# eniac/otti

Hardware: AMD Instinct MI355X
Metric: R1CS constraints/sec proved (Spartan NIZK) at 2^20 (higher is better)
Workload: dtype u256 (GF(l) / GF(2^255-19), 8 x u32 limbs)

## Files before the change

### include/otti_spartan.h

```cpp
#ifndef OTTI_SPARTAN_H
#define OTTI_SPARTAN_H
#include <stdint.h>
#include <stddef.h>

#ifdef __cplusplus
extern "C" {
#endif

enum {
    OTTI_OK = 0,
    OTTI_ERR_NON_POW2_CONS = -1,
    OTTI_ERR_NON_POW2_VARS = -2,
    OTTI_ERR_INVALID_NUM_INPUTS = -3,
    OTTI_ERR_INVALID_NUM_VARS = -4,
    OTTI_ERR_INVALID_SCALAR = -5,
    OTTI_ERR_INVALID_INDEX = -6,
    OTTI_ERR_VERIFY_INTERNAL = -10,
    OTTI_ERR_VERIFY_DECOMPRESS = -11,
    OTTI_ERR_MALFORMED_PROOF = -12,
    OTTI_ERR_NO_DEVICE = -20,
    OTTI_ERR_BAD_ARG = -21,
    OTTI_ERR_IO = -22,
    OTTI_ERR_INTERNAL = -23
};
// ... 123 lines not shown
                              uint8_t *io_Az, uint8_t *io_Bz, uint8_t *io_Cz, uint64_t *io_bits, uint64_t *io_unsat,
                              uint32_t *h_rows, size_t n_rows_cap, uint64_t *n_touched, int32_t *took_full_pass, float *kernel_ms);
int32_t otti_k_eval_table_sparse(otti_instance *inst, const uint8_t *h_eq_rx, const uint8_t *h_rABC , uint8_t *h_out, float *kernel_ms);
typedef struct { uint64_t rows, entries[3], n_heavy, n_seg; int32_t use_small, quad; } otti_device_info;
int32_t otti_instance_device_info(otti_instance *inst, int32_t by_col, otti_device_info *out);
int32_t otti_k_eq_evals(const uint8_t *h_r, size_t ell, uint8_t *h_out, float *kernel_ms);
int32_t otti_k_fold_top(const uint8_t *h_Z, size_t len, const uint8_t *h_r, uint8_t *h_out, float *kernel_ms);
int32_t otti_k_fold_bot(const uint8_t *h_Z, size_t len, const uint8_t *h_r, uint8_t *h_out, float *kernel_ms);
int32_t otti_k_sc_cubic_round(const uint8_t *h_A, const uint8_t *h_B, const uint8_t *h_C, const uint8_t *h_D, size_t len, uint8_t *h_e3, float *kernel_ms);
int32_t otti_k_sc_cubic_fold_round(const uint8_t *h_A, const uint8_t *h_B, const uint8_t *h_C, const uint8_t *h_D, size_t len,
                                   const uint8_t *h_r, uint8_t *h_out4, uint8_t *h_e3, float *kernel_ms);
int32_t otti_k_sc_quad_round(const uint8_t *h_A, const uint8_t *h_B, size_t len, uint8_t *h_e2, float *kernel_ms);
int32_t otti_k_sc_quad_fold_round(const uint8_t *h_A, const uint8_t *h_B, size_t len, const uint8_t *h_r, uint8_t *h_out2, uint8_t *h_e2, float *kernel_ms);
int32_t otti_k_armed_selftest(const uint8_t *A, const uint8_t *B, size_t len, const uint8_t *r, uint32_t hold_us, uint8_t *out2, uint8_t *e2);
int32_t otti_k_msm_rows(otti_gens *gens, const uint8_t *h_Z, size_t L, size_t R, const uint8_t *h_blinds, uint8_t *h_out32, float *kernel_ms);
int32_t otti_k_msm_scatter_rows(otti_gens *gens, size_t L, const uint64_t *h_idx, const uint8_t *h_s, size_t count,
                                uint8_t *h_out32, float *kernel_ms);
int32_t otti_k_witness_diff(const uint8_t *h_old, size_t n, const void *h_src, int32_t format, size_t stride_bytes, uint8_t *h_new,
                            uint64_t *h_idx, uint8_t *h_delta, uint64_t *n_changed, uint32_t *chunk, float *kernel_ms);
int32_t otti_k_row_sum(const uint8_t *h_compressed32, size_t n, const uint8_t *h_scalars_mont32, uint8_t *h_out32);

int32_t otti_k_eq_pyramid(const uint8_t *h_r, size_t n, uint8_t *h_out);
int32_t otti_k_sc_cubic3_round(const uint8_t *h_B, const uint8_t *h_C, const uint8_t *h_D, size_t len, const uint8_t *h_tau, uint8_t *h_e3, float *kernel_ms);
int32_t otti_k_sc_cubic3_fold_round(const uint8_t *h_B, const uint8_t *h_C, const uint8_t *h_D, size_t len, const uint8_t *h_r, const uint8_t *h_tau,
                                    uint8_t *h_out3, uint8_t *h_e3, float *kernel_ms);
int32_t otti_k_poly_bound(const uint8_t *h_Z, size_t L, size_t R, const uint8_t *h_Lv, uint8_t *h_out, float *kernel_ms);
int32_t otti_k_bullet_round(otti_gens *gens, size_t n_cur, int32_t fold, const uint8_t *h_u, const uint8_t *h_uinv, const uint8_t *h_a, const uint8_t *h_b,
                            const uint8_t *h_s, const uint8_t *h_blinds2, uint8_t *h_a_out, uint8_t *h_b_out, uint8_t *h_s_out, uint8_t *h_LR64, float *kernel_ms);
int32_t otti_k_bullet_last_fold(size_t R, const uint8_t *h_u, const uint8_t *h_uinv, uint8_t *h_a2, uint8_t *h_b2, uint8_t *h_s);
int32_t otti_k_pc_round(const uint8_t *h_A, const uint8_t *h_B, const uint8_t *h_C, const uint8_t *h_has_C, size_t ninst, size_t len, const uint8_t *h_tau,
// ... 48 lines not shown
```

### otti_amd/api.py

```python
import contextlib
import ctypes
import os
import sys
import numpy as np

L_ORDER = 2 ** 252 + 27742317777372353535851937790883648493
_R = (1 << 256) % L_ORDER
_RINV = pow(_R, -1, L_ORDER)

ENTRY_DTYPE = np.dtype([("row", "<u8"), ("col", "<u8"), ("val", "u1", (32,))])

_HERE = os.path.dirname(os.path.abspath(__file__))
lib_path = os.path.join(_HERE, "libottispartan.so")


class SpartanError(Exception):
    def __init__(self, code, msg=""):
        super().__init__(f"{type(self).__name__}({code}): {msg}")
        self.code = code


class R1CSError(SpartanError):
    """upstream R1CSError: InvalidNumberOfInputs(-3) InvalidNumberOfVars(-4) InvalidScalar(-5) InvalidIndex(-6)"""

# ... 122 lines not shown
_sig("otti_k_addr_timestamps", _i32, _vp, _sz, _sz, _vp, _vp, _fp)
_sig("otti_k_fr_to_canonical", _i32, _vp, _vp, _sz)
_sig("otti_k_multiply_vec", _i32, _vp, _vp, _vp, _vp, _vp, _fp)
_sig("otti_k_eval_table_sparse", _i32, _vp, _vp, _vp, _vp, _fp)
_sig("otti_k_products_patch", _i32, _vp, _vp, _vp, _sz, _sz, _sz, _vp, _vp, _vp, _vp, ctypes.POINTER(_u64), _vp, _sz, ctypes.POINTER(_u64), ctypes.POINTER(_i32), _fp)
_sig("otti_instance_device_info", _i32, _vp, _i32, ctypes.POINTER(_DeviceInfo))
_sig("otti_k_eq_evals", _i32, _vp, _sz, _vp, _fp)
_sig("otti_k_fold_top", _i32, _vp, _sz, _vp, _vp, _fp)
_sig("otti_k_fold_bot", _i32, _vp, _sz, _vp, _vp, _fp)
_sig("otti_k_sc_cubic_round", _i32, _vp, _vp, _vp, _vp, _sz, _vp, _fp)
_sig("otti_k_sc_cubic_fold_round", _i32, _vp, _vp, _vp, _vp, _sz, _vp, _vp, _vp, _fp)
_sig("otti_k_sc_quad_round", _i32, _vp, _vp, _sz, _vp, _fp)
_sig("otti_k_sc_quad_fold_round", _i32, _vp, _vp, _sz, _vp, _vp, _vp, _fp)
_sig("otti_k_armed_selftest", _i32, _vp, _vp, _sz, _vp, ctypes.c_uint32, _vp, _vp)
_sig("otti_k_msm_rows", _i32, _vp, _vp, _sz, _sz, _vp, _vp, _fp)
_sig("otti_k_row_sum", _i32, _vp, _sz, _vp, _vp)
_sig("otti_k_msm_scatter_rows", _i32, _vp, _sz, _vp, _vp, _sz, _vp, _fp)
_sig("otti_k_witness_diff", _i32, _vp, _sz, _vp, _i32, _sz, _vp, _vp, _vp, ctypes.POINTER(_u64), ctypes.POINTER(ctypes.c_uint32), _fp)
_sig("otti_k_eq_pyramid", _i32, _vp, _sz, _vp)
_sig("otti_k_sc_cubic3_round", _i32, _vp, _vp, _vp, _sz, _vp, _vp, _fp)
_sig("otti_k_sc_cubic3_fold_round", _i32, _vp, _vp, _vp, _sz, _vp, _vp, _vp, _vp, _fp)
_sig("otti_k_poly_bound", _i32, _vp, _sz, _sz, _vp, _vp, _fp)
_sig("otti_k_bullet_round", _i32, _vp, _sz, _i32, _vp, _vp, _vp, _vp, _vp, _vp, _vp, _vp, _vp, _vp, _fp)
_sig("otti_k_bullet_last_fold", _i32, _sz, _vp, _vp, _vp, _vp, _vp)
_u32 = ctypes.c_uint32
_sig("otti_k_pc_round", _i32, _vp, _vp, _vp, _vp, _sz, _sz, _vp, _vp, _u32, _u32, _vp, _vp, _fp)
_sig("otti_k_pc_export", _i32, _vp, _vp, _vp, _vp, _sz, _sz, _vp, _vp)
_sig("otti_k_pc_tail", _i32, _vp, _vp, _vp, _vp, _sz, _sz, _u32, _sz, _vp, _vp, _vp, _i32, _vp, _vp)
_sig("otti_k_prod_layer", _i32, _vp, _vp, _sz, _sz, _vp, _vp, _fp)
_sig("otti_k_hash_mem", _i32, _vp, _vp, _sz, _vp, _vp, _u32, _u32, _vp, _vp, _fp)
# ... 884 lines not shown
            raise ValueError("src is shorter than n elements at this stride")
        new, idx, delta = np.zeros((n, 32), dtype=np.uint8), np.zeros(n, dtype=np.uint64), np.zeros((n, 32), dtype=np.uint8)
        k, chunk = _u64(), ctypes.c_uint32()
        _check(lib.otti_k_witness_diff(_ptr(old), n, _ptr(raw), fmt, stride_bytes, _ptr(new), _ptr(idx), _ptr(delta), ctypes.byref(k), ctypes.byref(chunk), None))
        return new, idx[:k.value].copy(), delta[:k.value].copy(), chunk.value

    @staticmethod
    def msm_rows(gens, Z, L, R, blinds):
        Z, blinds = _scalars(Z, "Z"), _scalars(blinds, "blinds")
        assert Z.shape[0] == L * R and blinds.shape[0] == L
        out = np.zeros((L, 32), dtype=np.uint8); ms = ctypes.c_float(0)
        _check(lib.otti_k_msm_rows(gens._h, _ptr(Z), L, R, _ptr(blinds), _ptr(out), ctypes.byref(ms)))
        return out, ms.value

    @staticmethod
    def eq_pyramid(r):
        r = _scalars(r, "r"); n = r.shape[0]
        out = np.zeros(((2 << n) - 1, 32), dtype=np.uint8)
        _check(lib.otti_k_eq_pyramid(_ptr(r), n, _ptr(out)))
        return out

    @staticmethod
    def sc_cubic3_round(B, C, D, tau):
        B, C, D, tau = (_scalars(x, "t") for x in (B, C, D, tau)); e = np.zeros((3, 32), dtype=np.uint8); ms = ctypes.c_float(0)
        assert (1 << (tau.shape[0] + 1)) == B.shape[0]
        _check(lib.otti_k_sc_cubic3_round(_ptr(B), _ptr(C), _ptr(D), B.shape[0], _ptr(tau), _ptr(e), ctypes.byref(ms)))
        return e, ms.value

    @staticmethod
    def sc_cubic3_fold_round(B, C, D, r, tau):
# ... 232 lines not shown
```

### otti_amd/csrc/capi_kernels.cpp

```cpp
#include "capi_common.h"

namespace {
struct Staged {
    DevBuf<Fr> d;
    Staged(DevCtx &c, const uint8_t *h, size_t n) : d(std::max<size_t>(1, n)) { if (n) OTTI_HIP(hipMemcpyAsync(d.p, h, n * sizeof(Fr), hipMemcpyHostToDevice, c.stream)); }
};
void download(DevCtx &c, uint8_t *h, const Fr *d, size_t n) { if (n) OTTI_HIP(hipMemcpyAsync(h, d, n * sizeof(Fr), hipMemcpyDeviceToHost, c.stream)); }
struct KTimer {
    DevCtx &c; float *out;
    KTimer(DevCtx &c_, float *o) : c(c_), out(o) { if (out) OTTI_HIP(hipEventRecord(c.ev0, c.stream)); }
    void stop() { if (out) { OTTI_HIP(hipEventRecord(c.ev1, c.stream)); OTTI_HIP(hipEventSynchronize(c.ev1)); OTTI_HIP(hipEventElapsedTime(out, c.ev0, c.ev1)); } }
};
struct EqPyramids {
    DevBuf<Fr> buf; size_t n_lo = 0, n_hi = 0;
    EqPyramids(DevCtx &c, const Fr *tau, size_t m) : buf(8192 + 16384) {
        n_lo = std::min<size_t>(m, 12); n_hi = m - n_lo;
        dev_eq_pyramid2(c, tau + n_hi, n_lo, buf.p, tau, n_hi, n_hi ? buf.p + 8192 : nullptr);
    }
    EqSrc top() const {
        EqSrc e; const size_t m = n_lo + n_hi;
        if (m <= n_lo) { e.hi = nullptr; e.lo = buf.p + (((size_t)1 << m) - 1); e.lo_bits = 0; }
        else { e.hi = buf.p + 8192 + (((size_t)1 << n_hi) - 1); e.lo = buf.p + (((size_t)1 << n_lo) - 1); e.lo_bits = (int)n_lo; }
        return e;
    }
// ... 235 lines not shown
        pt_encode(out32, sum); return OTTI_OK;
    });
}
int32_t otti_k_msm_rows(otti_gens *gens, const uint8_t *Z, size_t L, size_t R, const uint8_t *blinds, uint8_t *out32, float *ms) {
    return guarded([&] {
        DevCtx &c = DevCtx::get(); Gens &g = *gens->g;
        if (R != g.R) throw Error(OTTI_ERR_BAD_ARG, "row length differs from the generator count");
        ensure_gens_device(g);
        Staged z(c, Z, L * R), bl(c, blinds, L);
        uint32_t hb = g.pc_n.h;
        const bool sparse = dev_small_fraction(c, z.d.p, L * R) > kSparseWitness;
        KTimer t(c, ms); dev_msm_rows(c, *g.dev, {.dense = z.d.p, .n_dense = R, .rows = L, .extra_s = bl.d.p, .extra_base = &hb, .n_extra = 1, .sparse = sparse}); t.stop();
        c.sync(); memcpy(out32, c.h_points, 32 * L); return OTTI_OK;
    });
}

int32_t otti_k_msm_scatter_rows(otti_gens *gens, size_t L, const uint64_t *idx, const uint8_t *s, size_t count, uint8_t *out32, float *ms) {
    return guarded([&] {
        if (!gens || !out32 || !L || L > 4096 || (count && (!idx || !s))) throw Error(OTTI_ERR_BAD_ARG, "null argument, or L outside 1 .. 4096");
        Gens &g = *gens->g;
        for (size_t i = 0; i < count; i++)
            if (idx[i] >= L * g.R || (i && idx[i] <= idx[i - 1])) throw Error(OTTI_ERR_INVALID_INDEX, "the indices are not strictly ascending below L * R");
        DevCtx &c = DevCtx::get();
        ensure_gens_device(g);
        Staged sc(c, s, count);
        DevBuf<uint64_t> d_idx(std::max<size_t>(1, count)); DevBuf<Pt> rows(L); DevBuf<uint8_t> enc(32 * L);
        const std::vector<Pt> id(L, pt_identity());
        if (count) OTTI_HIP(hipMemcpyAsync(d_idx.p, idx, count * sizeof(uint64_t), hipMemcpyHostToDevice, c.stream));
        OTTI_HIP(hipMemcpyAsync(rows.p, id.data(), L * sizeof(Pt), hipMemcpyHostToDevice, c.stream));
        KTimer t(c, ms); dev_msm_scatter(c, *g.dev, d_idx.p, sc.d.p, count, g.R, rows.p, L); t.stop();
// ... 358 lines not shown
```

### otti_amd/csrc/device.h

```cpp
#pragma once
#include <hip/hip_runtime.h>
#include <vector>
#include <functional>
#include <cstddef>
#include <chrono>
#include "spartan.h"
#include "mail.h"
#include "msm_plan.h"
#include "sc_plan.h"

namespace otti {

#define OTTI_HIP(expr) ::otti::hip_check((expr), #expr, __FILE__, __LINE__)
void hip_check(hipError_t e, const char *what, const char *file, int line);
struct OutOfDeviceMemory : Error { using Error::Error; };
struct TailTimeout : Error { using Error::Error; };

template <class T> struct DevBuf {
    T *p = nullptr; size_t n = 0;
    DevBuf() {}
    explicit DevBuf(size_t count) { alloc(count); }
    DevBuf(const DevBuf &) = delete; DevBuf &operator=(const DevBuf &) = delete;
    DevBuf(DevBuf &&o) noexcept : p(o.p), n(o.n) { o.p = nullptr; o.n = 0; }
    DevBuf &operator=(DevBuf &&o) noexcept { if (this != &o) { release(); p = o.p; n = o.n; o.p = nullptr; o.n = 0; } return *this; }
// ... 233 lines not shown
void dev_fold_bot(DevCtx &c, const Fr *Z, Fr *out, size_t len, const Fr &r);
void dev_fetch(DevCtx &c, const Fr *src, int slot, size_t n);
struct MsmJob {
    const Fr *dense = nullptr; size_t n_dense = 0, rows = 0;
    const Fr *extra_s = nullptr; const uint32_t *extra_base = nullptr ; size_t n_extra = 0;
    int mode = MSM_COMPRESSED;
    const Pt *addend = nullptr;
    bool sparse = false;
    Pt *keep_dst = nullptr; bool force_bulk = false;
};
constexpr double kSparseWitness = 0.25;
MsmTicket dev_msm_rows(DevCtx &c, const DeviceGens &g, const MsmJob &job);
double dev_small_fraction(DevCtx &c, const Fr *z, size_t n);
void dev_msm_scatter(DevCtx &c, const DeviceGens &g, const uint64_t *d_idx, const Fr *d_s, size_t count, size_t R, Pt *rows, size_t L);
void dev_encode_points(DevCtx &c, const Pt *pts, size_t n, uint8_t *d_out32);
void dev_poly_bound(DevCtx &c, const Fr *Z, size_t L, size_t R, const Fr *Lv, Fr *out, Fr *scratch );
bool dev_poly_bound_chunks(DevCtx &c, const Fr *Z, size_t L, size_t R, const Fr *Lv_rest, size_t m, Fr *out, Fr *scratch );
void dev_dot(DevCtx &c, const Fr *a, const Fr *b, size_t n, int slot);
void dev_bullet_step(DevCtx &c, Fr *a, Fr *b, Fr *s, size_t R, size_t n_cur, bool fold_first, const Fr &u, const Fr &u_inv, Fr *rows, Fr *extra_out);
void dev_bullet_finish(DevCtx &c, Fr *a, Fr *b, Fr *s, size_t R, const Fr &u, const Fr &u_inv, const Fr &d, Fr *rows, int slot_a);
struct BulletRound {
    size_t R, n_cur; bool fold; Fr u, u_inv;
    const Fr *a_in, *b_in, *s_in; Fr *a_out, *b_out, *s_out;
    const Fr *extra_s; const uint32_t *extra_base; bool armed = false;
};
MsmTicket dev_bullet_round(DevCtx &c, const DeviceGens &g, const BulletRound &round);
void dev_decode_niels(DevCtx &c, const uint8_t *compressed_dev, size_t n, Niels *out, unsigned *bad);
int dev_msm_var(DevCtx &c, const Niels *pts, const Fr *scalars, size_t n, Pt *out, size_t out_cap, int *n_windows, int *n_splits);
double dev_madd_peak(DevCtx &c);
void dev_fr_to_lanes(hipStream_t st, const Fr *d_src, const Fr *factor, unsigned long long *d_lanes, size_t n);
// ... 6 lines not shown
```

### otti_amd/csrc/k_msm.hip

```cpp
#include "kernels_common.h"

namespace otti {

constexpr int kMsmMaxChunk = 1024;
constexpr int kMsmBulkChunk = 512;
constexpr int kMsmListCap = (kMsmBulkChunk + 8) * 16;
static_assert(kMsmBulkChunk + 8 <= 2048, "work-list entries pack the term index (within a sub-chunk) in 11 bits");
__device__ __attribute__((noinline)) Fr fr_mul_shared(Fr a, Fr b) { return fr_mul(a, b); }
struct BulletArgs { int on, fold; uint32_t n; const Fr *a_in, *b_in, *s_in; Fr *a_out, *b_out, *s_out; Fr u, uinv, u_raw, uinv_raw; };
struct MsmArgs {
    const TabEntry *table; int c, W; uint32_t E; int lanes;
    const Fr *dense; size_t stride, n_dense; uint32_t chunk, nchunks;
    const Fr *extra_s; uint32_t extra_base[8]; int n_extra;
    uint32_t K[9];
    Pt *partial;
    int fuse; uint32_t rows; unsigned *counter; Pt *host_pts; unsigned long long *host_flag; unsigned long long seq; MsmMail *mail;
    BulletArgs bul;
    Armed go;
    unsigned long long *stamps;
};
__device__ __forceinline__ Fr bullet_fold_a(const BulletArgs &U, size_t x) { return U.fold ? fr_add(fr_mul_shared(U.a_in[x], U.u), fr_mul_shared(U.uinv, U.a_in[U.n + x])) : U.a_in[x]; }
__device__ __forceinline__ Fr bullet_fold_b(const BulletArgs &U, size_t x) { return U.fold ? fr_add(fr_mul_shared(U.b_in[x], U.uinv), fr_mul_shared(U.u, U.b_in[U.n + x])) : U.b_in[x]; }
__device__ __forceinline__ size_t bullet_slot(const BulletArgs &U, size_t row, size_t t) {
    const size_t n = U.n, h = n / 2;
// ... 1 lines not shown
}
__device__ __forceinline__ Fr bullet_fold_s(const BulletArgs &U, size_t j) { return U.fold ? fr_mul_shared(U.s_in[j], ((j & (2 * (size_t)U.n - 1)) < U.n) ? U.uinv : U.u) : U.s_in[j]; }
__device__ __forceinline__ void recode_scalar(uint32_t *dst9, const Fr &sc, const uint32_t (&K)[9]) {
    const Fr raw = fr_to_raw(sc);
    uint64_t cy = 0;
#pragma unroll
    for (int i = 0; i < 8; i++) { cy += (uint64_t)raw.v[i] + K[i]; dst9[i] = (uint32_t)cy; cy >>= 32; }
    dst9[8] = (uint32_t)cy + K[8];
}
__device__ __forceinline__ int recoded_digit(const uint32_t *src9, int w, int c) {
    const int pos = w * c, limb = pos >> 5, off = pos & 31;
    uint64_t x = src9[limb];
    if (limb < 8) x |= (uint64_t)src9[limb + 1] << 32;
    return (int)((uint32_t)(x >> off) & ((1u << c) - 1u)) - (1 << (c - 1));
}
enum { MSM_BULK = 0, MSM_SMALL = 1, MSM_BULK_SPARSE = 2 };
template <int kKind> __global__ __launch_bounds__(kBlock) void k_msm_rows(MsmArgs A) {
    static_assert(kKind == MSM_BULK || kKind == MSM_BULK_SPARSE, "small launches use k_msm_small");
    constexpr size_t kRawBytes = ((kKind == MSM_BULK_SPARSE ? kMsmBulkChunk : kMsmMaxChunk) + 8) * 9 * sizeof(uint32_t), kTreeBytes = (kBlock / 2) * sizeof(P10);
    __shared__ __attribute__((aligned(16))) unsigned char s_mem[kRawBytes > kTreeBytes ? kRawBytes : kTreeBytes];
    __shared__ uint32_t s_base[8];
    uint32_t *s_raw = reinterpret_cast<uint32_t *>(s_mem);
    P10 *sm = reinterpret_cast<P10 *>(s_mem);
    const size_t row = blockIdx.y; const uint32_t chunk_id = blockIdx.x;
    const size_t j0 = (size_t)chunk_id * A.chunk;
    const uint32_t n_here = (uint32_t)min((size_t)A.chunk, A.n_dense - j0);
    const uint32_t n_ex = chunk_id == 0 ? (uint32_t)A.n_extra : 0u;
    if (threadIdx.x < 8) s_base[threadIdx.x] = A.extra_base[threadIdx.x];
    __syncthreads();
    P9 acc9 = p9_identity();
    const int w = threadIdx.x % A.W, tl = threadIdx.x / A.W;
    if constexpr (kKind == MSM_BULK_SPARSE) {
        __shared__ uint16_t s_list[kMsmListCap];
        __shared__ uint32_t s_count;
        const uint32_t n_all = n_here + n_ex;
        const int pos = w * A.c, limb = pos >> 5, off = pos & 31;
        const uint32_t mask = (1u << A.c) - 1u; const int half = 1 << (A.c - 1);
        const unsigned lane = threadIdx.x & 63;
        const size_t WE = (size_t)A.W * A.E;
        const uint32_t sub_cap = min((uint32_t)kMsmBulkChunk, (uint32_t)(kMsmListCap / A.W));
        for (uint32_t sub0 = 0; sub0 < n_all; sub0 += sub_cap) {
            const uint32_t n_tot = min(sub_cap, n_all - sub0), iters = (n_tot + A.lanes - 1) / A.lanes;
            __syncthreads();
            for (uint32_t t = threadIdx.x; t < n_tot; t += blockDim.x) {
                const uint32_t T = sub0 + t;
                const Fr sc = T >= n_here ? A.extra_s[row * A.n_extra + (T - n_here)] : A.dense[row * A.stride + j0 + T];
                recode_scalar(s_raw + t * 9, sc, A.K);
            }
            if (threadIdx.x == 0) s_count = 0;
            __syncthreads();
            for (uint32_t it = 0; it < iters; it++) {
                const uint32_t t = (uint32_t)tl + it * (uint32_t)A.lanes;
                bool nz = false;
                if (tl < A.lanes && t < n_tot) {
                    uint64_t x = s_raw[t * 9 + limb];
                    if (limb < 8) x |= (uint64_t)s_raw[t * 9 + limb + 1] << 32;
                    nz = ((uint32_t)(x >> off) & mask) != (uint32_t)half;
                }
                const unsigned long long bal = __ballot(nz);
                uint32_t base_pos = 0;
                if (lane == 0 && bal) base_pos = atomicAdd(&s_count, (uint32_t)__popcll(bal));
                base_pos = __shfl(base_pos, 0);
                if (nz) s_list[base_pos + __popcll(bal & ((1ull << lane) - 1ull))] = (uint16_t)((t << 5) | (uint32_t)w);
            }
            __syncthreads();
// ... 8 lines not shown
                acc9 = p9_madd(acc9, e);
            }
        }
    } else {
        const size_t WE = (size_t)A.W * A.E;
        const uint32_t n_all = n_here + n_ex;
        for (uint32_t sub0 = 0; sub0 < n_all; sub0 += kMsmMaxChunk) {
            const uint32_t n_tot = min((uint32_t)kMsmMaxChunk, n_all - sub0);
            if (sub0) __syncthreads();
            for (uint32_t t = threadIdx.x; t < n_tot; t += blockDim.x) {
                const uint32_t T = sub0 + t;
                const Fr sc = T >= n_here ? A.extra_s[row * A.n_extra + (T - n_here)] : A.dense[row * A.stride + j0 + T];
                recode_scalar(s_raw + t * 9, sc, A.K);
            }
            __syncthreads();
            if (tl < A.lanes)
                for (uint32_t t = tl; t < n_tot; t += A.lanes) {
                    const int d = recoded_digit(s_raw + t * 9, w, A.c);
                    if (d == 0) continue;
                    const uint32_t T = sub0 + t;
                    size_t base = T < n_here ? j0 + T : (size_t)s_base[T - n_here];
                    uint32_t mag = (uint32_t)(d < 0 ? -d : d);
                    N9 e = n9_unpack(A.table[base * WE + (size_t)w * A.E + (mag - 1)].n);
                    if (d < 0) e = n9_negate(e);
                    acc9 = p9_madd(acc9, e);
                }
        }
    }
    __syncthreads();
    P10 acc = p10_unpack(p9_pack(acc9));
    const F10 d2 = f10_const(fp_2D());
    for (int sft = kBlock / 2; sft >= 1; sft >>= 1) {
        if ((int)threadIdx.x >= sft && (int)threadIdx.x < 2 * sft) sm[threadIdx.x - sft] = acc;
        __syncthreads();
        if ((int)threadIdx.x < sft) acc = p10_add(acc, sm[threadIdx.x], d2);
        __syncthreads();
    }
    if (threadIdx.x == 0) A.partial[row * A.nchunks + chunk_id] = p10_pack(acc);
}

constexpr int kMsmScatterSub = 256;
struct MsmScatterArgs {
    const TabEntry *table; int c, W; uint32_t E; int lanes; uint32_t K[9];
    const unsigned long long *idx; const Fr *s; size_t count, R; Pt *rows;
};
__device__ __forceinline__ size_t scatter_lower_bound(const unsigned long long *idx, size_t n, unsigned long long key) {
    size_t lo = 0, hi = n;
    while (lo < hi) { const size_t mid = lo + (hi - lo) / 2; if (idx[mid] < key) lo = mid + 1; else hi = mid; }
    return lo;
}
__global__ __launch_bounds__(kBlock) void k_msm_scatter(MsmScatterArgs A) {
    constexpr size_t kRawBytes = (size_t)kMsmScatterSub * 9 * sizeof(uint32_t), kTreeBytes = (kBlock / 2) * sizeof(P10);
    __shared__ __attribute__((aligned(16))) unsigned char s_mem[kRawBytes > kTreeBytes ? kRawBytes : kTreeBytes];
// ... 240 lines not shown
    if (i >= n) return;
    P10 p = p10_unpack(pts[i]);
    if (addend) p = p10_add(p, p10_unpack(addend[i]), f10_const(fp_2D()));
    uint8_t enc[32]; p10_encode(enc, p);
    uint32_t w[8];
    for (int k = 0; k < 8; k++) w[k] = (uint32_t)enc[4 * k] | ((uint32_t)enc[4 * k + 1] << 8) | ((uint32_t)enc[4 * k + 2] << 16) | ((uint32_t)enc[4 * k + 3] << 24);
    uint32_t *o = (uint32_t *)(out32 + 32 * i);
    for (int k = 0; k < 8; k++) o[k] = w[k];
    if (host32) { uint32_t *h = (uint32_t *)(host32 + 32 * i); for (int k = 0; k < 8; k++) h[k] = w[k]; }
}
void dev_encode_points(DevCtx &c, const Pt *pts, size_t n, uint8_t *d_out32) {
    if (!n) return;
    KScope ks(c, KC_MSM_FINISH);
    hipLaunchKernelGGL(k_encode_points, (unsigned)((n + 63) / 64), 64, 0, c.stream, pts, (const Pt *)nullptr, n, d_out32, (uint8_t *)nullptr);
}
__global__ __launch_bounds__(kBlock) void k_count_small(const Fr *z, size_t n, unsigned long long *count) {
    unsigned mine = 0;
    for (size_t i = blockIdx.x * (size_t)blockDim.x + threadIdx.x; i < n; i += (size_t)gridDim.x * blockDim.x) {
        Fr r = fr_to_raw(z[i]);
        mine += (r.v[4] | r.v[5] | r.v[6] | r.v[7]) == 0 ? 1u : 0u;
    }
    for (int o = 32; o >= 1; o >>= 1) mine += __shfl_down(mine, o);
    if ((threadIdx.x & 63) == 0 && mine) atomicAdd(count, (unsigned long long)mine);
}
double dev_small_fraction(DevCtx &c, const Fr *z, size_t n) {
    if (!n) return 0.0;
    const Tallies t = counted_launch(c, [&](unsigned long long *count) { hipLaunchKernelGGL(k_count_small, grid_for(n), kBlock, 0, c.stream, z, n, count); });
    return (double)t.first / (double)n;
}
static void msm_report_stamps(DevCtx &c, const unsigned long long *t, const MsmJob &j, const MsmPlan &p, bool bullet) {
    OTTI_HIP(hipStreamSynchronize(c.stream));
    auto us = [&](int a, int b) { return t[b] >= t[a] ? (double)(t[b] - t[a]) * 0.01 : -1.0; };
    const size_t rows = j.rows, terms = j.n_dense + j.n_extra, nchunks = p.nchunks;
    if (p.route == MsmRoute::mail) {
        const auto h0 = std::chrono::steady_clock::now();
        c.msm_host_sum(c.msm_mail.pending[c.msm_mail.pending_n - 1]);
        const double host_us = std::chrono::duration<double, std::micro>(std::chrono::steady_clock::now() - h0).count();
        fprintf(stderr, "[otti] k_msm_small rows=%zu terms=%zu chunks=%zu bullet=%d host-sum: scalars %.2f | pairs %.2f | tree + mail %.2f | total %.2f us on the device; "
                        "host sum of %zu mails (all in) %.2f us\n",
                rows, terms, nchunks, bullet ? 1 : 0, us(0, 1), us(1, 2), us(2, 3), us(0, 3), rows * nchunks, host_us);
    } else
        fprintf(stderr, "[otti] k_msm_small rows=%zu terms=%zu chunks=%zu bullet=%d: scalars %.2f | pairs %.2f | tree %.2f | (others arrive) %.2f | chunk sums %.2f | row tree %.2f | mail %.2f | total %.2f us\n",
                rows, terms, nchunks, bullet ? 1 : 0, us(0, 1), us(1, 2), us(2, 3), us(3, 4), us(4, 5), us(5, 6), us(6, 7), us(0, 7));
}
static MsmTicket msm_launch(DevCtx &c, const DeviceGens &g, const MsmJob &j, const BulletArgs *bul) {
    if (j.n_extra > 8) throw Error(OTTI_ERR_INTERNAL, "msm: too many extra terms");
    const size_t rows = j.rows;
    if (!rows) return {};
    const MsmPlan p = msm_plan({g.c, g.W, rows, j.n_dense, j.n_extra, bul != nullptr, j.mode, j.addend != nullptr, j.sparse, j.force_bulk, c.msm_mail.host_sum(c)});
    const size_t nchunks = p.nchunks;
    if (p.route == MsmRoute::raw && rows > kHostPtsCap) throw Error(OTTI_ERR_INTERNAL, "msm: too many raw rows");
    MsmArgs A;
    A.table = g.table.p; A.c = g.c; A.W = g.W; A.E = (uint32_t)g.E; A.lanes = kBlock / g.W;
    A.dense = j.dense; A.stride = j.n_dense; A.n_dense = j.n_dense; A.extra_s = j.extra_s; A.n_extra = (int)j.n_extra;
    for (int i = 0; i < 8; i++) A.extra_base[i] = i < (int)j.n_extra ? j.extra_base[i] : 0;
    A.chunk = (uint32_t)p.chunk; A.nchunks = (uint32_t)nchunks;
    for (int i = 0; i < 9; i++) A.K[i] = p.K[i];
    c.ensure_points(rows, nchunks);
    A.partial = c.msm_partial.p;
    A.fuse = p.fuse;
    if (p.route == MsmRoute::mail) c.msm_mail.ensure(c);
    if (bul) A.bul = *bul; else { memset(&A.bul, 0, sizeof A.bul); }
    A.go = Armed{nullptr, nullptr, 0};
    A.rows = (uint32_t)rows; A.counter = c.d_counter2.p; A.host_pts = c.d_pts_alias; A.host_flag = c.d_flag_alias; A.seq = A.fuse ? ++c.seq : 0;
    A.mail = A.fuse == 2 ? c.msm_mail.dev + (size_t)(c.msm_mail.launches % kMsmMailRegions) * kMsmMailCap : nullptr;
    static const bool want_stamps = getenv("OTTI_MSM_STAMPS") != nullptr;
    static thread_local unsigned long long *h_stamps = nullptr, *d_stamps = nullptr;
    A.stamps = nullptr;
    if (want_stamps && A.fuse) {
        if (!h_stamps) { OTTI_HIP(hipHostMalloc((void **)&h_stamps, 128, hipHostMallocDefault)); OTTI_HIP(hipHostGetDevicePointer((void **)&d_stamps, h_stamps, 0)); }
        memset(h_stamps, 0, 128); A.stamps = d_stamps;
    }
    if (bul && bul->on == 2) { A.bul.on = 1; if (!A.stamps) A.go = c.arm(); else throw Error(OTTI_ERR_INTERNAL, "armed launches cannot be stamped"); }
    {
        const dim3 grid((unsigned)nchunks, (unsigned)rows);
        KScope ks(c, p.kernel == MsmKernel::small ? KC_MSM_SMALL : KC_MSM_ROWS);
        if (p.kernel == MsmKernel::bulk_sparse) hipLaunchKernelGGL(k_msm_rows<MSM_BULK_SPARSE>, grid, kBlock, 0, c.stream, A);
        else if (p.kernel == MsmKernel::bulk) hipLaunchKernelGGL(k_msm_rows<MSM_BULK>, grid, kBlock, 0, c.stream, A);
        else hipLaunchKernelGGL(k_msm_small, grid, kBlock, 0, c.stream, A);
    }
    const MsmTicket ticket{A.seq, (uint32_t)rows, p.route};
    if (p.route == MsmRoute::mail) c.msm_mail.queue(A.seq, (uint32_t)rows, (uint32_t)nchunks);
    if (A.stamps) msm_report_stamps(c, h_stamps, j, p, bul != nullptr);
    c.pending_host_encode = p.route == MsmRoute::mail || p.route == MsmRoute::flag || p.route == MsmRoute::host_encode ? rows : 0;
    if (ticket.delivers_without_sync()) return ticket;
    c.msm_mail.h_pts_order = ++c.msm_mail.order;
    const Pt *finals = c.msm_partial.p;
    if (nchunks > 1) {
        KScope ks(c, KC_MSM_FINISH);
        hipLaunchKernelGGL(k_msm_finish, (unsigned)rows, 64, 0, c.stream, (const Pt *)c.msm_partial.p, (uint32_t)nchunks, rows, c.msm_final.p);
        finals = c.msm_final.p;
    }
    if (p.route == MsmRoute::keep) {
        if (!j.keep_dst && c.msm_keep.n < rows) c.msm_keep.alloc(rows);
        OTTI_HIP(hipMemcpyAsync(j.keep_dst ? j.keep_dst : c.msm_keep.p, finals, rows * sizeof(Pt), hipMemcpyDeviceToDevice, c.stream));
    } else if (p.route == MsmRoute::device_encode) {
        KScope ks(c, KC_MSM_FINISH);
        hipLaunchKernelGGL(k_encode_points, (unsigned)((rows + 63) / 64), 64, 0, c.stream, finals, j.addend, rows, c.d_points.p, c.d_points_host);
        if (!c.d_points_host) OTTI_HIP(hipMemcpyAsync(c.h_points, c.d_points.p, rows * 32, hipMemcpyDeviceToHost, c.stream));
    } else OTTI_HIP(hipMemcpyAsync(c.h_pts, finals, rows * sizeof(Pt), hipMemcpyDeviceToHost, c.stream));
    return ticket;
}
MsmTicket dev_msm_rows(DevCtx &c, const DeviceGens &g, const MsmJob &job) {
    if (job.keep_dst && job.mode != MSM_KEEP) throw Error(OTTI_ERR_INTERNAL, "msm: a destination for kept row sums needs MSM_KEEP");
    return msm_launch(c, g, job, nullptr);
}
MsmTicket dev_bullet_round(DevCtx &c, const DeviceGens &g, const BulletRound &r) {
    BulletArgs U; U.on = r.armed ? 2 : 1; U.fold = r.fold ? 1 : 0; U.n = (uint32_t)r.n_cur; U.a_in = r.a_in; U.b_in = r.b_in; U.s_in = r.s_in;
    U.a_out = r.a_out; U.b_out = r.b_out; U.s_out = r.s_out; U.u = r.u; U.uinv = r.u_inv; U.u_raw = fr_to_raw(r.u); U.uinv_raw = fr_to_raw(r.u_inv);
    return msm_launch(c, g, {.n_dense = r.R / 2, .rows = 2, .extra_s = r.extra_s, .extra_base = r.extra_base, .n_extra = 2}, &U);
}
// ... 217 lines not shown
```

### otti_amd/csrc/prover.cpp

```cpp
#include "device.h"
#include "pool.h"
#include "shard.h"
#include <chrono>
#include <cstring>
#include <mutex>

namespace otti {

constexpr size_t kHostTailBits = 5;
constexpr int kTailSlot = 64;

static double now_ms() { return std::chrono::duration<double, std::milli>(std::chrono::steady_clock::now().time_since_epoch()).count(); }

int device_window_bits(size_t nbases) {
    if (const char *e = getenv("OTTI_MSM_WINDOW")) { int c = atoi(e); if (c >= 4 && c <= 17) return c; }
    double budget_gb = 200.0;
    if (const char *e = getenv("OTTI_MSM_TABLE_GB")) { double v = atof(e); if (v > 0) budget_gb = v; }
    int best = 8;
    const int widest = nbases < 256 ? 12 : 17;
    for (int c = 8; c <= widest; c++) {
        const double W = 253 / c + 1, bytes = (double)nbases * W * (double)((size_t)1 << (c - 1)) * sizeof(TabEntry);
        if (bytes <= budget_gb * 1073741824.0) best = c;
    }
    return best;
// ... 342 lines not shown
    for (int k = 0; k < 2; k++)
        for (auto &p : st[k]->pre) { p.delta = c.h_pts[row]; p.bp_h = c.h_pts[row + 1]; p.be_h = c.h_pts[row + 2]; p.rb_h = c.h_pts[row + 3]; p.to_fe(); row += 4; }
    std::vector<RoundPre *> all; for (int k = 0; k < 2; k++) for (auto &p : st[k]->pre) all.push_back(&p);
    SpinPool &pool = SpinPool::get(); const int nt = pool.workers() + 1;
    std::vector<std::function<void()>> tasks(nt);
    for (int t = 0; t < nt; t++) tasks[t] = [&, t] { for (size_t j = t; j < all.size(); j += nt) pt_encode(all[j]->delta_c.b, all[j]->delta); };
    pool.parallel(tasks.data(), nt);
}
struct ProofScratch {
    size_t N = 0, V = 0;
    DevBuf<Fr> T[4];
    DevBuf<Fr> zw, ABC;
    DevBuf<Fr> eqs;
    DevBuf<Fr> pyr;
    DevBuf<Fr> blinds, Lv, Rv, LZ, a, s, b2, s2, rows, extras, bound_scratch, pre;
    void reserve(size_t n, size_t v, size_t Lsz, size_t Rsz, size_t lgR) {
        if (n == N && v == V) return;
        for (auto &t : T) t.alloc(n);
        zw.alloc(2 * v); ABC.alloc(2 * v); eqs.alloc(5 * 4096); pyr.alloc(8192 + 16384);
        blinds.alloc(Lsz); Lv.alloc(Lsz); Rv.alloc(Rsz); LZ.alloc(Rsz); a.alloc(Rsz); s.alloc(Rsz); b2.alloc(Rsz); s2.alloc(Rsz); rows.alloc(2 * Rsz);
        extras.alloc(4 * (lgR + 1)); bound_scratch.alloc(64 * Rsz);
        N = n; V = v;
    }
};
}
struct Scratch : ProofScratch {};
namespace {
ProofScratch &workspace(DevCtx &c) { if (!c.scratch) c.scratch = new Scratch(); return *c.scratch; }

inline CPoint point_at(const DevCtx &c, size_t i) { CPoint p; memcpy(p.b, c.h_points + 32 * i, 32); return p; }
// ... 165 lines not shown
        std::vector<std::pair<const char *, size_t>> sched;
        auto sumcheck_sched = [&](size_t rounds, size_t ne) {
            sched.push_back({"blinds_poly", rounds}); sched.push_back({"blinds_evals", rounds});
            for (size_t j = 0; j < rounds; j++) { sched.push_back({"d_vec", ne}); sched.push_back({"r_delta", 1}); sched.push_back({"r_beta", 1}); }
        };
        auto drawn = [&] { size_t n = 0; for (auto &e : sched) n += e.second; return n; };
        sched.push_back({"poly_blinds", Lsz});
        off_sc1 = drawn(); sumcheck_sched(nrx, 4);
        for (const char *l : {"Az_blind", "Bz_blind", "Cz_blind", "prod_Az_Bz_blind", "t1", "t2", "b1", "b2", "b3", "b4", "b5", "r"}) sched.push_back({l, 1});
        off_sc2 = drawn(); sumcheck_sched(nry, 3);
        sched.push_back({"blind_eval", 1}); sched.push_back({"d", 1}); sched.push_back({"r_delta", 2});
        sched.push_back({"blinds_vec_1", 2 * lgR}); sched.push_back({"blinds_vec_2", 2 * lgR}); sched.push_back({"r", 1});
        tape.prefetch(sched);
    }
    std::vector<Fr> blinds_vars = tape.random_vector("poly_blinds", Lsz);
    OTTI_HIP(hipMemcpyAsync(S.blinds.p, blinds_vars.data() + rk * Ll, Ll * sizeof(Fr), hipMemcpyHostToDevice, c.stream));
    {
        uint32_t hbase = g.pc_n.h;
        dev_msm_rows(c, DG, {.rows = Ll, .extra_s = S.blinds.p, .extra_base = &hbase, .n_extra = 1, .addend = rows_kept ? wit.rows_kept.p : c.msm_keep.p});
        OTTI_HIP(hipEventRecord(c.ev0, c.stream));
        if (!sh && wit.products_kept_for(I))
            for (int k = 0; k < 3; k++) OTTI_HIP(hipMemcpyAsync(S.T[1 + k].p, wit.prod_abc[k].p, N * sizeof(Fr), hipMemcpyDeviceToDevice, c.stream));
        else dev_spmv3(c, rows_set, wit.z.p, S.T[1].p, S.T[2].p, S.T[3].p, false, nullptr);
        { RandomTape::Cursor c1(tape, off_sc1), c2(tape, off_sc2); sumcheck_draw_tape(early1, c1, nrx, 4); sumcheck_draw_tape(early2, c2, nry, 3); }
        round_points = precompute_round_points_launch(c, DG, g, early1, early2, S.pre);
        OTTI_HIP(hipEventSynchronize(c.ev0));
        P.comm_vars.resize(Lsz);
        static_assert(sizeof(CPoint) == 32, "CPoint is 32 packed bytes");
        if (sh) sh->allgather(c.h_points, Ll * 32, P.comm_vars.data());
        else for (size_t i = 0; i < Lsz; i++) P.comm_vars[i] = point_at(c, i);
        tr.append_message("poly_commitment", "poly_commitment_begin", 21);
        for (auto &cp : P.comm_vars) tr.append_point("poly_commitment_share", cp.b);
        tr.append_message("poly_commitment", "poly_commitment_end", 19);
    }
// ... 240 lines not shown
```

Before: 386.4 million.

## Add fused commit-tail kernel for blind term plus kept row sums

Adds a dedicated k_commit_tail kernel that, for each row, adds the blind scalar times the hiding base to the kept MSM row sum and encodes the point in one launch. The prover uses it in place of a second generic msm_rows pass when there are many rows, reading the blinds from pinned host memory instead of an explicit copy. The MSM row kernel also gets a quad-lane cooperative tree reduction, and when there is a single chunk it writes kept results straight into the keep buffer, dropping a device-to-device copy. Optional timestamp probes are added as well. The risk is mainly more code paths, and the device reading blinds over the host link.

```diff
diff --git a/include/otti_spartan.h b/include/otti_spartan.h
--- a/include/otti_spartan.h
+++ b/include/otti_spartan.h
@@ -161,6 +161,7 @@
 int32_t otti_k_sc_quad_fold_round(const uint8_t *h_A, const uint8_t *h_B, size_t len, const uint8_t *h_r, uint8_t *h_out2, uint8_t *h_e2, float *kernel_ms);
 int32_t otti_k_armed_selftest(const uint8_t *A, const uint8_t *B, size_t len, const uint8_t *r, uint32_t hold_us, uint8_t *out2, uint8_t *e2);
 int32_t otti_k_msm_rows(otti_gens *gens, const uint8_t *h_Z, size_t L, size_t R, const uint8_t *h_blinds, uint8_t *h_out32, float *kernel_ms);
+int32_t otti_k_commit_rows_two_step(otti_gens *gens, const uint8_t *h_Z, size_t L, size_t R, const uint8_t *h_blinds, uint8_t *h_out32, float *kernel_ms);
 int32_t otti_k_msm_scatter_rows(otti_gens *gens, size_t L, const uint64_t *h_idx, const uint8_t *h_s, size_t count,
                                 uint8_t *h_out32, float *kernel_ms);
 int32_t otti_k_witness_diff(const uint8_t *h_old, size_t n, const void *h_src, int32_t format, size_t stride_bytes, uint8_t *h_new,
diff --git a/otti_amd/api.py b/otti_amd/api.py
--- a/otti_amd/api.py
+++ b/otti_amd/api.py
@@ -160,6 +160,7 @@
 _sig("otti_k_sc_quad_fold_round", _i32, _vp, _vp, _sz, _vp, _vp, _vp, _fp)
 _sig("otti_k_armed_selftest", _i32, _vp, _vp, _sz, _vp, ctypes.c_uint32, _vp, _vp)
 _sig("otti_k_msm_rows", _i32, _vp, _vp, _sz, _sz, _vp, _vp, _fp)
+_sig("otti_k_commit_rows_two_step", _i32, _vp, _vp, _sz, _sz, _vp, _vp, _fp)
 _sig("otti_k_row_sum", _i32, _vp, _sz, _vp, _vp)
 _sig("otti_k_msm_scatter_rows", _i32, _vp, _sz, _vp, _vp, _sz, _vp, _fp)
 _sig("otti_k_witness_diff", _i32, _vp, _sz, _vp, _i32, _sz, _vp, _vp, _vp, ctypes.POINTER(_u64), ctypes.POINTER(ctypes.c_uint32), _fp)
@@ -1074,6 +1075,14 @@
         return out, ms.value
 
     @staticmethod
+    def commit_rows_two_step(gens, Z, L, R, blinds):
+        Z, blinds = _scalars(Z, "Z"), _scalars(blinds, "blinds")
+        assert Z.shape[0] == L * R and blinds.shape[0] == L
+        out = np.zeros((L, 32), dtype=np.uint8); ms = ctypes.c_float(0)
+        _check(lib.otti_k_commit_rows_two_step(gens._h, _ptr(Z), L, R, _ptr(blinds), _ptr(out), ctypes.byref(ms)))
+        return out, ms.value
+
+    @staticmethod
     def eq_pyramid(r):
         r = _scalars(r, "r"); n = r.shape[0]
         out = np.zeros(((2 << n) - 1, 32), dtype=np.uint8)
diff --git a/otti_amd/csrc/capi_kernels.cpp b/otti_amd/csrc/capi_kernels.cpp
--- a/otti_amd/csrc/capi_kernels.cpp
+++ b/otti_amd/csrc/capi_kernels.cpp
@@ -273,6 +273,23 @@
         c.sync(); memcpy(out32, c.h_points, 32 * L); return OTTI_OK;
     });
 }
+int32_t otti_k_commit_rows_two_step(otti_gens *gens, const uint8_t *Z, size_t L, size_t R, const uint8_t *blinds, uint8_t *out32, float *ms) {
+    return guarded([&] {
+        DevCtx &c = DevCtx::get(); Gens &g = *gens->g;
+        if (!Z || !blinds || !out32 || !L) throw Error(OTTI_ERR_BAD_ARG, "null argument or no rows");
+        if (R != g.R) throw Error(OTTI_ERR_BAD_ARG, "row length differs from the generator count");
+        ensure_gens_device(g);
+        Staged z(c, Z, L * R), bl(c, blinds, L);
+        uint32_t hb = g.pc_n.h;
+        const bool sparse = dev_small_fraction(c, z.d.p, L * R) > kSparseWitness;
+        KTimer t(c, ms);
+        dev_msm_rows(c, *g.dev, {.dense = z.d.p, .n_dense = R, .rows = L, .mode = MSM_KEEP, .sparse = sparse});
+        if (L > kHostEncodeRows) dev_commit_tail(c, *g.dev, bl.d.p, hb, c.msm_keep.p, L);
+        else dev_msm_rows(c, *g.dev, {.rows = L, .extra_s = bl.d.p, .extra_base = &hb, .n_extra = 1, .addend = c.msm_keep.p});
+        t.stop();
+        c.sync(); memcpy(out32, c.h_points, 32 * L); return OTTI_OK;
+    });
+}
 
 int32_t otti_k_msm_scatter_rows(otti_gens *gens, size_t L, const uint64_t *idx, const uint8_t *s, size_t count, uint8_t *out32, float *ms) {
     return guarded([&] {
diff --git a/otti_amd/csrc/device.h b/otti_amd/csrc/device.h
--- a/otti_amd/csrc/device.h
+++ b/otti_amd/csrc/device.h
@@ -271,6 +271,7 @@
 double dev_small_fraction(DevCtx &c, const Fr *z, size_t n);
 void dev_msm_scatter(DevCtx &c, const DeviceGens &g, const uint64_t *d_idx, const Fr *d_s, size_t count, size_t R, Pt *rows, size_t L);
 void dev_encode_points(DevCtx &c, const Pt *pts, size_t n, uint8_t *d_out32);
+void dev_commit_tail(DevCtx &c, const DeviceGens &g, const Fr *blinds, uint32_t base, const Pt *addend, size_t rows);
 void dev_poly_bound(DevCtx &c, const Fr *Z, size_t L, size_t R, const Fr *Lv, Fr *out, Fr *scratch );
 bool dev_poly_bound_chunks(DevCtx &c, const Fr *Z, size_t L, size_t R, const Fr *Lv_rest, size_t m, Fr *out, Fr *scratch );
 void dev_dot(DevCtx &c, const Fr *a, const Fr *b, size_t n, int slot);
diff --git a/otti_amd/csrc/k_msm.hip b/otti_amd/csrc/k_msm.hip
--- a/otti_amd/csrc/k_msm.hip
+++ b/otti_amd/csrc/k_msm.hip
@@ -39,6 +39,28 @@
     if (limb < 8) x |= (uint64_t)src9[limb + 1] << 32;
     return (int)((uint32_t)(x >> off) & ((1u << c) - 1u)) - (1 << (c - 1));
 }
+__device__ __forceinline__ F10 msm_tree256(const P10 &acc, P10 *sm) {
+    const F10 d2 = f10_const(fp_2D());
+    const int t = threadIdx.x, q = t & 3, qid = t >> 2;
+    if (t >= kBlock / 2) sm[t - kBlock / 2] = acc;
+    __syncthreads();
+    if (t < kBlock / 2) sm[t] = p10_add(acc, sm[t], d2);
+    __syncthreads();
+    F10 *const smf = reinterpret_cast<F10 *>(sm);
+    F10 a = smf[4 * qid + q];
+    const F10 b = smf[4 * (qid + kBlock / 4) + q];
+    __syncthreads();
+    a = q10_add_cached(a, q10_cached(q10_u(b, q), q, d2), q);
+#pragma unroll 1
+    for (int sft = kBlock / 8; sft >= 1; sft >>= 1) {
+        const F10 ua = q10_u(a, q);
+        F10 *const level = smf + 4 * (sft - 1) + q;
+        if (qid >= sft && qid < 2 * sft) level[4 * (qid - sft)] = q10_cached(ua, q, d2);
+        __syncthreads();
+        if (qid < sft) a = q10_add_cached_u(ua, level[4 * qid], q);
+    }
+    return a;
+}
 enum { MSM_BULK = 0, MSM_SMALL = 1, MSM_BULK_SPARSE = 2 };
 template <int kKind> __global__ __launch_bounds__(kBlock) void k_msm_rows(MsmArgs A) {
     static_assert(kKind == MSM_BULK || kKind == MSM_BULK_SPARSE, "small launches use k_msm_small");
@@ -51,6 +73,8 @@
     const size_t j0 = (size_t)chunk_id * A.chunk;
     const uint32_t n_here = (uint32_t)min((size_t)A.chunk, A.n_dense - j0);
     const uint32_t n_ex = chunk_id == 0 ? (uint32_t)A.n_extra : 0u;
+    const bool stamp0 = A.stamps && threadIdx.x == 0 && blockIdx.x == 0 && blockIdx.y == 0;
+    if (stamp0) A.stamps[0] = wall_clock64();
     if (threadIdx.x < 8) s_base[threadIdx.x] = A.extra_base[threadIdx.x];
     __syncthreads();
     P9 acc9 = p9_identity();
@@ -74,6 +98,7 @@
             }
             if (threadIdx.x == 0) s_count = 0;
             __syncthreads();
+            if (stamp0 && !sub0) A.stamps[1] = wall_clock64();
             for (uint32_t it = 0; it < iters; it++) {
                 const uint32_t t = (uint32_t)tl + it * (uint32_t)A.lanes;
                 bool nz = false;
@@ -112,6 +137,7 @@
                 recode_scalar(s_raw + t * 9, sc, A.K);
             }
             __syncthreads();
+            if (stamp0 && !sub0) A.stamps[1] = wall_clock64();
             if (tl < A.lanes)
                 for (uint32_t t = tl; t < n_tot; t += A.lanes) {
                     const int d = recoded_digit(s_raw + t * 9, w, A.c);
@@ -126,15 +152,10 @@
         }
     }
     __syncthreads();
-    P10 acc = p10_unpack(p9_pack(acc9));
-    const F10 d2 = f10_const(fp_2D());
-    for (int sft = kBlock / 2; sft >= 1; sft >>= 1) {
-        if ((int)threadIdx.x >= sft && (int)threadIdx.x < 2 * sft) sm[threadIdx.x - sft] = acc;
-        __syncthreads();
-        if ((int)threadIdx.x < sft) acc = p10_add(acc, sm[threadIdx.x], d2);
-        __syncthreads();
-    }
-    if (threadIdx.x == 0) A.partial[row * A.nchunks + chunk_id] = p10_pack(acc);
+    if (stamp0) A.stamps[2] = wall_clock64();
+    const F10 sum = msm_tree256(p10_unpack(p9_pack(acc9)), sm);
+    if (threadIdx.x < 4) reinterpret_cast<Fp *>(&A.partial[row * A.nchunks + chunk_id])[threadIdx.x] = f10_pack(sum);
+    if (stamp0) A.stamps[3] = wall_clock64();
 }
 
 constexpr int kMsmScatterSub = 256;
@@ -405,6 +426,69 @@
     KScope ks(c, KC_MSM_FINISH);
     hipLaunchKernelGGL(k_encode_points, (unsigned)((n + 63) / 64), 64, 0, c.stream, pts, (const Pt *)nullptr, n, d_out32, (uint8_t *)nullptr);
 }
+constexpr int kTailBlock = 64, kTailQuads = kTailBlock / 4;
+struct CommitTailArgs { const TabEntry *column; int c, W; uint32_t E; uint32_t K[9]; const Fr *blinds; const Pt *addend; size_t rows; uint8_t *out32, *host32; };
+__global__ __launch_bounds__(kTailBlock) void k_commit_tail(CommitTailArgs A) {
+    __shared__ uint32_t s_raw[kTailQuads][9];
+    const int q = threadIdx.x & 3, qid = threadIdx.x >> 2;
+    const size_t row = (size_t)blockIdx.x * kTailQuads + qid;
+    const bool live = row < A.rows;
+    if (live && q == 0) recode_scalar(s_raw[qid], A.blinds[row], A.K);
+    __syncthreads();
+    if (!live) return;
+    const uint32_t *mine = s_raw[qid];
+    const Fp kept_w = reinterpret_cast<const Fp *>(&A.addend[row])[q];
+    F10 acc = q10_identity(q);
+    Fp nxt; bool nxt_have = false, nxt_neg = false;
+    auto fetch = [&](int w) {
+        const int d = recoded_digit(mine, w, A.c);
+        nxt_have = d != 0;
+        if (!nxt_have) return;
+        nxt_neg = d < 0;
+        const Niels *e = &A.column[(size_t)w * A.E + ((uint32_t)(d < 0 ? -d : d) - 1)].n;
+        if (q < 3) nxt = reinterpret_cast<const Fp *>(e)[q == 2 ? 2 : (((q == 0) != nxt_neg) ? 1 : 0)];
+    };
+    fetch(0);
+#pragma unroll 1
+    for (int w = 0; w < A.W; w++) {
+        const Fp cur = nxt; const bool have = nxt_have, neg = nxt_neg;
+        if (w + 1 < A.W) fetch(w + 1);
+        if (!have) continue;
+        F10 v;
+        if (q == 3) { v = f10_zero(); v.v[0] = 2; }
+        else { v = f10_unpack(cur); if (q == 2 && neg) v = f10_carry(f10_neg(v)); }
+        acc = q10_add_cached(acc, v, q);
+    }
+    const F10 kept = f10_unpack(kept_w);
+    acc = q10_add_cached(acc, q10_cached(q10_u(kept, q), q, f10_const(fp_2D())), q);
+    P10 p;
+    p.X = f10_quad_perm<F10_QP(0, 0, 0, 0)>(acc); p.Y = f10_quad_perm<F10_QP(1, 1, 1, 1)>(acc);
+    p.Z = f10_quad_perm<F10_QP(2, 2, 2, 2)>(acc); p.T = f10_quad_perm<F10_QP(3, 3, 3, 3)>(acc);
+    uint8_t enc[32]; p10_encode(enc, p);
+    if (q) return;
+    uint32_t *o = (uint32_t *)(A.out32 + 32 * row), *h = A.host32 ? (uint32_t *)(A.host32 + 32 * row) : nullptr;
+    for (int k = 0; k < 8; k++) {
+        const uint32_t wd = (uint32_t)enc[4 * k] | ((uint32_t)enc[4 * k + 1] << 8) | ((uint32_t)enc[4 * k + 2] << 16) | ((uint32_t)enc[4 * k + 3] << 24);
+        o[k] = wd;
+        if (h) h[k] = wd;
+    }
+}
+void dev_commit_tail(DevCtx &c, const DeviceGens &g, const Fr *blinds, uint32_t base, const Pt *addend, size_t rows) {
+    if (!rows) return;
+    if (!blinds || !addend || base >= g.nbases) throw Error(OTTI_ERR_INTERNAL, "commit tail: no blinds, no kept sums, or a base beyond the table");
+    c.ensure_points(rows, 1);
+    CommitTailArgs A;
+    A.column = g.entry0(base); A.c = g.c; A.W = g.W; A.E = (uint32_t)g.E;
+    msm_recoding_constant(A.K, g.c, g.W);
+    A.blinds = blinds; A.addend = addend; A.rows = rows; A.out32 = c.d_points.p; A.host32 = c.d_points_host;
+    {
+        KScope ks(c, KC_MSM_FINISH);
+        hipLaunchKernelGGL(k_commit_tail, (unsigned)((rows + kTailQuads - 1) / kTailQuads), kTailBlock, 0, c.stream, A);
+    }
+    if (!c.d_points_host) OTTI_HIP(hipMemcpyAsync(c.h_points, c.d_points.p, rows * 32, hipMemcpyDeviceToHost, c.stream));
+    c.pending_host_encode = 0;
+    c.msm_mail.h_pts_order = ++c.msm_mail.order;
+}
 __global__ __launch_bounds__(kBlock) void k_count_small(const Fr *z, size_t n, unsigned long long *count) {
     unsigned mine = 0;
     for (size_t i = blockIdx.x * (size_t)blockDim.x + threadIdx.x; i < n; i += (size_t)gridDim.x * blockDim.x) {
@@ -423,7 +507,10 @@
     OTTI_HIP(hipStreamSynchronize(c.stream));
     auto us = [&](int a, int b) { return t[b] >= t[a] ? (double)(t[b] - t[a]) * 0.01 : -1.0; };
     const size_t rows = j.rows, terms = j.n_dense + j.n_extra, nchunks = p.nchunks;
-    if (p.route == MsmRoute::mail) {
+    if (p.kernel != MsmKernel::small)
+        fprintf(stderr, "[otti] k_msm_rows<%d> rows=%zu terms=%zu chunks=%zu, workgroup (0, 0): first recode %.2f | phase 2 %.2f | phase 3 %.2f | total %.2f us\n",
+                p.kernel == MsmKernel::bulk_sparse ? 2 : 0, rows, terms, nchunks, us(0, 1), us(1, 2), us(2, 3), us(0, 3));
+    else if (p.route == MsmRoute::mail) {
         const auto h0 = std::chrono::steady_clock::now();
         c.msm_host_sum(c.msm_mail.pending[c.msm_mail.pending_n - 1]);
         const double host_us = std::chrono::duration<double, std::micro>(std::chrono::steady_clock::now() - h0).count();
@@ -448,7 +535,12 @@
     A.chunk = (uint32_t)p.chunk; A.nchunks = (uint32_t)nchunks;
     for (int i = 0; i < 9; i++) A.K[i] = p.K[i];
     c.ensure_points(rows, nchunks);
-    A.partial = c.msm_partial.p;
+    Pt *keep = nullptr;
+    if (p.route == MsmRoute::keep) {
+        if (!j.keep_dst && c.msm_keep.n < rows) c.msm_keep.alloc(rows);
+        keep = j.keep_dst ? j.keep_dst : c.msm_keep.p;
+    }
+    A.partial = keep && nchunks == 1 ? keep : c.msm_partial.p;
     A.fuse = p.fuse;
     if (p.route == MsmRoute::mail) c.msm_mail.ensure(c);
     if (bul) A.bul = *bul; else { memset(&A.bul, 0, sizeof A.bul); }
@@ -458,7 +550,7 @@
     static const bool want_stamps = getenv("OTTI_MSM_STAMPS") != nullptr;
     static thread_local unsigned long long *h_stamps = nullptr, *d_stamps = nullptr;
     A.stamps = nullptr;
-    if (want_stamps && A.fuse) {
+    if (want_stamps && (A.fuse || p.kernel != MsmKernel::small)) {
         if (!h_stamps) { OTTI_HIP(hipHostMalloc((void **)&h_stamps, 128, hipHostMallocDefault)); OTTI_HIP(hipHostGetDevicePointer((void **)&d_stamps, h_stamps, 0)); }
         memset(h_stamps, 0, 128); A.stamps = d_stamps;
     }
@@ -479,13 +571,11 @@
     const Pt *finals = c.msm_partial.p;
     if (nchunks > 1) {
         KScope ks(c, KC_MSM_FINISH);
-        hipLaunchKernelGGL(k_msm_finish, (unsigned)rows, 64, 0, c.stream, (const Pt *)c.msm_partial.p, (uint32_t)nchunks, rows, c.msm_final.p);
+        hipLaunchKernelGGL(k_msm_finish, (unsigned)rows, 64, 0, c.stream, (const Pt *)c.msm_partial.p, (uint32_t)nchunks, rows, keep ? keep : c.msm_final.p);
         finals = c.msm_final.p;
     }
-    if (p.route == MsmRoute::keep) {
-        if (!j.keep_dst && c.msm_keep.n < rows) c.msm_keep.alloc(rows);
-        OTTI_HIP(hipMemcpyAsync(j.keep_dst ? j.keep_dst : c.msm_keep.p, finals, rows * sizeof(Pt), hipMemcpyDeviceToDevice, c.stream));
-    } else if (p.route == MsmRoute::device_encode) {
+    if (p.route == MsmRoute::keep) return ticket;
+    if (p.route == MsmRoute::device_encode) {
         KScope ks(c, KC_MSM_FINISH);
         hipLaunchKernelGGL(k_encode_points, (unsigned)((rows + 63) / 64), 64, 0, c.stream, finals, j.addend, rows, c.d_points.p, c.d_points_host);
         if (!c.d_points_host) OTTI_HIP(hipMemcpyAsync(c.h_points, c.d_points.p, rows * 32, hipMemcpyDeviceToHost, c.stream));
diff --git a/otti_amd/csrc/prover.cpp b/otti_amd/csrc/prover.cpp
--- a/otti_amd/csrc/prover.cpp
+++ b/otti_amd/csrc/prover.cpp
@@ -380,6 +380,15 @@
     DevBuf<Fr> eqs;
     DevBuf<Fr> pyr;
     DevBuf<Fr> blinds, Lv, Rv, LZ, a, s, b2, s2, rows, extras, bound_scratch, pre;
+    Fr *h_blinds = nullptr, *h_blinds_dev = nullptr; size_t h_blinds_n = 0;
+    bool pin_blinds(size_t n) {
+        if (h_blinds_n >= n) return h_blinds_dev != nullptr;
+        if (h_blinds) (void)hipHostFree(h_blinds);
+        h_blinds = h_blinds_dev = nullptr; h_blinds_n = n;
+        if (hipHostMalloc((void **)&h_blinds, n * sizeof(Fr), hipHostMallocDefault) != hipSuccess) { (void)hipGetLastError(); h_blinds = nullptr; return false; }
+        if (hipHostGetDevicePointer((void **)&h_blinds_dev, h_blinds, 0) != hipSuccess) { (void)hipGetLastError(); h_blinds_dev = nullptr; }
+        return h_blinds_dev != nullptr;
+    }
     void reserve(size_t n, size_t v, size_t Lsz, size_t Rsz, size_t lgR) {
         if (n == N && v == V) return;
         for (auto &t : T) t.alloc(n);
@@ -575,10 +584,14 @@
         tape.prefetch(sched);
     }
     std::vector<Fr> blinds_vars = tape.random_vector("poly_blinds", Lsz);
-    OTTI_HIP(hipMemcpyAsync(S.blinds.p, blinds_vars.data() + rk * Ll, Ll * sizeof(Fr), hipMemcpyHostToDevice, c.stream));
+    const Fr *d_blinds = S.blinds.p;
+    if (Ll > kHostEncodeRows && S.pin_blinds(Ll)) { memcpy(S.h_blinds, blinds_vars.data() + rk * Ll, Ll * sizeof(Fr)); d_blinds = S.h_blinds_dev; }
+    else OTTI_HIP(hipMemcpyAsync(S.blinds.p, blinds_vars.data() + rk * Ll, Ll * sizeof(Fr), hipMemcpyHostToDevice, c.stream));
     {
         uint32_t hbase = g.pc_n.h;
-        dev_msm_rows(c, DG, {.rows = Ll, .extra_s = S.blinds.p, .extra_base = &hbase, .n_extra = 1, .addend = rows_kept ? wit.rows_kept.p : c.msm_keep.p});
+        const Pt *kept = rows_kept ? wit.rows_kept.p : c.msm_keep.p;
+        if (Ll > kHostEncodeRows) dev_commit_tail(c, DG, d_blinds, hbase, kept, Ll);
+        else dev_msm_rows(c, DG, {.rows = Ll, .extra_s = S.blinds.p, .extra_base = &hbase, .n_extra = 1, .addend = kept});
         OTTI_HIP(hipEventRecord(c.ev0, c.stream));
         if (!sh && wit.products_kept_for(I))
             for (int k = 0; k < 3; k++) OTTI_HIP(hipMemcpyAsync(S.T[1 + k].p, wit.prod_abc[k].p, N * sizeof(Fr), hipMemcpyDeviceToDevice, c.stream));
```

After: 383.4 million. No clear change (-0.8%).
